# tomguluson92/SCAT

Measured on AMD Instinct MI355X. Metric: images/sec (train step, 256x256 source -> 224x224, reg_transformer), higher is better.
Workload: dtype f32; 1 GPU; ResNet-50 + dim-halving transformer (8 heads) + 3 regressor iterations, pl_reg, mask_rate 0.2, pos_embed, Adam; full train step (BASELINE configs[1]); batch_per_gpu=96, global_batch=96, parallelism=dp1

## Files before the change

### scat_amd/_lib.py

```python
from __future__ import annotations

import ctypes
import os
import re

HERE = os.path.dirname(os.path.abspath(__file__))
HEADER = os.path.join(HERE, "..", "include", "scat_hip.h")
EVAL_HEADER = os.path.join(HERE, "..", "include", "scat_eval.h")
RENDER_HEADER = os.path.join(HERE, "..", "include", "scat_render.h")
MANO_HEADER = os.path.join(HERE, "..", "include", "scat_mano.h")
FIT_HEADER = os.path.join(HERE, "..", "include", "scat_mano_fit.h")
FIT_KP_HEADER = os.path.join(HERE, "..", "include", "scat_mano_fit_kp.h")
HEADERS = (HEADER, EVAL_HEADER, FIT_KP_HEADER, FIT_HEADER, RENDER_HEADER, MANO_HEADER)
LIBPATH = os.path.join(HERE, "libscat_hip.so")
if os.environ.get("SCAT_LIBPATH"):
    import warnings

    LIBPATH = os.path.abspath(os.environ["SCAT_LIBPATH"])
    warnings.warn(f"scat_amd: SCAT_LIBPATH set, loading {LIBPATH} instead of the shipped libscat_hip.so", RuntimeWarning)

_CT = {
    "int": ctypes.c_int,
    "int64_t": ctypes.c_int64,
    "uint64_t": ctypes.c_uint64,
    "float": ctypes.c_float,
}


def parse_header(path: str = HEADER):
    src = open(path).read()
    src = re.sub(r"/\*.*?\*/", "", src, flags=re.S)
    src = re.sub(r"//[^\n]*", "", src)
    protos = {}
    for m in re.finditer(r"(?m)^\s*(const char\*|int64_t|int)\s+(scat_\w+)\s*\(([^;{]*?)\)\s*;", src, flags=re.S):
        ret, name, args = m.group(1), m.group(2), " ".join(m.group(3).split())
        at = []
        if args and args != "void":
            for a in args.split(","):
                a = a.strip()
                if "*" in a:
                    at.append((ctypes.c_void_p, a.split("*")[-1].strip()))
                else:
                    ty, an = a.rsplit(" ", 1)
                    at.append((_CT[ty.replace("const ", "").strip()], an))
        rt = {"int": ctypes.c_int, "int64_t": ctypes.c_int64, "const char*": ctypes.c_char_p}[ret]
        protos[name] = (rt, at)
# ... 53 lines not shown
```

### scat_amd/build.py

```python
from __future__ import annotations

import os
import subprocess
import sys
from concurrent.futures import ThreadPoolExecutor

HERE = os.path.dirname(os.path.abspath(__file__))
CSRC = os.path.join(HERE, "csrc")
OUT = os.path.join(HERE, "libscat_hip.so")
OBJ = os.path.join(HERE, "csrc", "_obj")
HIPCC = os.environ.get("HIPCC", "/opt/rocm/bin/hipcc")
FLAGS = ["-O3", "--offload-arch=gfx950", "-fPIC", "-std=c++17", "-fno-slp-vectorize", "-Wall", "-Wno-unused-function",
         "-Wno-unused-variable"]


def _sources():
    return sorted(f for f in os.listdir(CSRC) if f.endswith(".hip"))


def _public_headers_mtime():
    return max(os.path.getmtime(os.path.join(HERE, "..", "include", h)) for h in ("scat_hip.h", "scat_eval.h", "scat_render.h", "scat_mano.h", "scat_mano_fit.h", "scat_mano_fit_kp.h"))


def _deps_mtime():
    m = 0.0
    for root, _, files in os.walk(CSRC):
        if root.endswith(("_obj", "_obj_diag")):
            continue
        for f in files:
            if f.endswith((".h", ".hip")):
                m = max(m, os.path.getmtime(os.path.join(root, f)))
    return max(m, _public_headers_mtime())


DIAG_OUT = os.path.join(HERE, "..", "tools", "_bin", "libscat_hip_diag.so")


def build(force: bool = False, verbose: bool = True, diag: bool = False) -> str:
    global OUT, OBJ
    if diag:
        out, obj, flags = os.path.abspath(DIAG_OUT), os.path.join(CSRC, "_obj_diag"), FLAGS + ["-DSCAT_DIAG"]
        os.makedirs(os.path.dirname(out), exist_ok=True)
        saved = (OUT, OBJ, list(FLAGS))
        OUT, OBJ = out, obj
        FLAGS[:] = flags
        try:
            return build(force, verbose, False)
        finally:
            OUT, OBJ = saved[0], saved[1]
            FLAGS[:] = saved[2]
    if not force and os.path.exists(OUT) and os.path.getmtime(OUT) >= _deps_mtime():
        return OUT
    os.makedirs(OBJ, exist_ok=True)
    hdr_m = max(os.path.getmtime(os.path.join(CSRC, f)) for f in os.listdir(CSRC) if f.endswith(".h"))
# ... 31 lines not shown
```

### scat_amd/csrc/norm.hip

```cpp
#include <atomic>
#include <chrono>

#include "common.h"

namespace scat {

__device__ __forceinline__ double wave_sum(double v) {
#pragma unroll
    for (int o = 32; o > 0; o >>= 1) v += __shfl_down(v, o, 64);
    return v;
}
__device__ __forceinline__ float wave_sum_f(float v) {
#pragma unroll
    for (int o = 32; o > 0; o >>= 1) v += __shfl_xor(v, o, 64);
    return v;
}

__device__ __forceinline__ void block_sum2(double& a, double& b, double* sh) {
    a = wave_sum(a);
    b = wave_sum(b);
    const int lane = threadIdx.x & 63, w = threadIdx.x >> 6;
    if (lane == 0) { sh[w] = a; sh[4 + w] = b; }
    __syncthreads();
    if (threadIdx.x == 0) {
        a = sh[0] + sh[1] + sh[2] + sh[3];
        b = sh[4] + sh[5] + sh[6] + sh[7];
    }
}

struct BnSlot {
    double s1, s2;
    unsigned long long tag, pad;
};
static std::atomic<unsigned long long> g_bn_tag{1};
static unsigned long long bn_next_tag() {
    static const unsigned long long salt =
// ... 364 lines not shown
    }
}

__global__ __launch_bounds__(256) void bn_bwd_pool_apply_kernel(const float* __restrict__ dyp, const int8_t* __restrict__ idx,
                                                                const float* __restrict__ x, int relu,
                                                                const float* __restrict__ scale,
                                                                const float* __restrict__ shift,
                                                                const float* __restrict__ mean,
                                                                const float* __restrict__ invstd,
                                                                const float* __restrict__ gamma,
                                                                const float* __restrict__ coef, float* __restrict__ dx,
                                                                int64_t total, int C, int W, int OH, int OW) {
    const int QW = OW / 2;
    for (int64_t e = blockIdx.x * 256ll + threadIdx.x; e < total; e += gridDim.x * 256ll) {
        const int b2 = e % QW;
        const int64_t r = e / QW;
        const int a = r % OH;
        const int64_t nc = r / OH;
        const int c = (int)(nc % C);
        const float* g = dyp + nc * OH * OW;
        const int8_t* id = idx + nc * OH * OW;
        const int b = 2 * b2;
        float gv[2][3];
        int iv[2][3];
#pragma unroll
        for (int u = 0; u < 2; ++u)
#pragma unroll
            for (int v = 0; v < 3; ++v) {
                const bool ok = (a + u < OH) && (b + v < OW);
                const int q = ok ? (a + u) * OW + b + v : 0;
                gv[u][v] = ok ? g[q] : 0.f;
                iv[u][v] = ok ? (int)id[q] : -1;
            }
        float top[4], bot[4];
#pragma unroll
        for (int v = 0; v < 2; ++v) {
            top[2 * v] = iv[0][v] == 4 ? gv[0][v] : 0.f;
            top[2 * v + 1] = (iv[0][v] == 5 ? gv[0][v] : 0.f) + (iv[0][v + 1] == 3 ? gv[0][v + 1] : 0.f);
            bot[2 * v] = (iv[0][v] == 7 ? gv[0][v] : 0.f) + (iv[1][v] == 1 ? gv[1][v] : 0.f);
            bot[2 * v + 1] = (iv[0][v] == 8 ? gv[0][v] : 0.f) + (iv[0][v + 1] == 6 ? gv[0][v + 1] : 0.f) +
                             (iv[1][v] == 2 ? gv[1][v] : 0.f) + (iv[1][v + 1] == 0 ? gv[1][v + 1] : 0.f);
        }
        const float sc = scale[c], sh = shift[c], mu = mean[c], is = invstd[c];
        const float k1 = coef[2 * c], k2 = coef[2 * c + 1], gi = gamma[c] * is;
        const int64_t off = (nc * 2 * OH + 2 * a) * W + 2 * b;
        const float4 x0 = *(const float4*)(x + off), x1 = *(const float4*)(x + off + W);
        const float xt[4] = {x0.x, x0.y, x0.z, x0.w}, xb[4] = {x1.x, x1.y, x1.z, x1.w};
        float ot[4], ob[4];
#pragma unroll
        for (int q = 0; q < 4; ++q) {
            const float gt = bn_mask(top[q], xt[q], 0.f, false, relu, sc, sh), gb = bn_mask(bot[q], xb[q], 0.f, false, relu, sc, sh);
            ot[q] = gi * (gt - k1 - (xt[q] - mu) * is * k2);
            ob[q] = gi * (gb - k1 - (xb[q] - mu) * is * k2);
        }
        *(float4*)(dx + off) = make_float4(ot[0], ot[1], ot[2], ot[3]);
        *(float4*)(dx + off + W) = make_float4(ob[0], ob[1], ob[2], ob[3]);
    }
}

template <int V>
__global__ __launch_bounds__(1024) void bn_bwd_reduce_fin_kernel(const float* __restrict__ dy, const float* __restrict__ x,
                                                                 const float* __restrict__ yout,
                                                                 const uint8_t* __restrict__ ymask, int relu,
                                                                 const float* __restrict__ scale,
                                                                 const float* __restrict__ shift,
                                                                 const float* __restrict__ mean,
                                                                 const float* __restrict__ invstd, int B, int C, int HW,
                                                                 FastDiv dHWv, double count, float* __restrict__ dgamma,
                                                                 float* __restrict__ dbeta, float* __restrict__ coef) {
    const int c = blockIdx.x;
    const float sc = scale[c], sh = shift[c], mu = mean[c], is = invstd[c];
    const int hwv = HW / V;
    const bool has_m = V == 4 && ymask != nullptr;
    const bool has_y = yout != nullptr || has_m;
    double s1 = 0, s2 = 0;
    for (int idx = threadIdx.x; idx < B * hwv; idx += 1024) {
        const int n = (int)dHWv.div((uint32_t)idx), i = idx - n * hwv;
        const int64_t off = ((int64_t)n * C + c) * HW + i * V;
        float xv[V], gv[V], yv[V];
        if (V == 4) {
            float4 t = ld4x(x + off); xv[0] = t.x; xv[1] = t.y; xv[2] = t.z; xv[3] = t.w;
            t = *(const float4*)(dy + off); gv[0] = t.x; gv[1] = t.y; gv[2] = t.z; gv[3] = t.w;
            if (has_m) {
                const uint32_t m = ymask[off >> 2];
                yv[0] = (float)(m & 1u); yv[1] = (float)((m >> 1) & 1u); yv[2] = (float)((m >> 2) & 1u); yv[3] = (float)((m >> 3) & 1u);
            } else if (has_y) { t = *(const float4*)(yout + off); yv[0] = t.x; yv[1] = t.y; yv[2] = t.z; yv[3] = t.w; }
// ... 551 lines not shown
                               shift, save_mean, save_invstd, B, C, HW, FastDiv::make(HW / 4), (double)B * HW, dgamma,
                               dbeta, coef);
        else
            hipLaunchKernelGGL(bn_bwd_reduce_fin_kernel<1>, dim3(C), dim3(1024), 0, st, dy, x, y_out, nullptr, relu, scale,
                               shift, save_mean, save_invstd, B, C, HW, FastDiv::make(HW), (double)B * HW, dgamma, dbeta,
                               coef);
    } else {
        BnFin f = bn_fin_base(ws, C, S, (double)B * HW);
        f.dgamma = dgamma; f.dbeta = dbeta; f.coef = coef; f.coef3 = 0;
        if (vec)
            hipLaunchKernelGGL(bn_bwd_reduce_kernel<4>, dim3(C, S), dim3(256), 0, st, dy, x, y_out, y_mask, relu, scale,
                               shift, save_mean, save_invstd, B, C, HW, S, FastDiv::make(HW / 4), part, f);
        else
            hipLaunchKernelGGL(bn_bwd_reduce_kernel<1>, dim3(C, S), dim3(256), 0, st, dy, x, y_out, nullptr, relu, scale,
                               shift, save_mean, save_invstd, B, C, HW, S, FastDiv::make(HW), part, f);
        if (!f.slots)
            hipLaunchKernelGGL(bn_bwd_finalize_kernel, dim3(cdiv(C, 128)), dim3(128), 0, st, (const double*)part, C, S,
                               (double)B * HW, dgamma, dbeta, coef);
    }
    if (vec) {
        const int64_t nv = total / 4;
        hipLaunchKernelGGL(bn_bwd_apply_kernel<4>, dim3(ew_grid(nv)), dim3(256), 0, st, dy, x, y_out, y_mask, relu,
                           scale, shift, save_mean, save_invstd, gamma, (const float*)coef, dx, dres, dres_accumulate, nv,
                           FastDiv::make(HW / 4), FastDiv::make(C), store_policy(total * 4) == 2);
    } else {
        hipLaunchKernelGGL(bn_bwd_apply_kernel<1>, dim3(ew_grid(total)), dim3(256), 0, st, dy, x, y_out, nullptr, relu,
                           scale, shift, save_mean, save_invstd, gamma, (const float*)coef, dx, dres, dres_accumulate, total,
                           FastDiv::make(HW), FastDiv::make(C), 0);
    }
    SCAT_LAUNCH_CHECK("scat_bn_bwd");
    return SCAT_OK;
}

extern "C" int scat_bn_bwd_maxpool(const float* dy_pooled, const int8_t* idx, const float* x, int relu, const float* scale,
                                   const float* shift, const float* save_mean, const float* save_invstd,
                                   const float* gamma, float* dgamma, float* dbeta, float* dx, int B, int C, int H, int W,
                                   void* ws, int64_t ws_bytes, void* stream) {
    SCAT_REQUIRE(dy_pooled && idx && x && scale && shift && save_mean && save_invstd && gamma && dgamma && dbeta && dx,
                 SCAT_E_ARG, "scat_bn_bwd_maxpool: null pointer");
    SCAT_REQUIRE(B > 0 && C > 0 && H > 0 && W > 0 && H % 2 == 0 && W % 4 == 0, SCAT_E_SHAPE,
                 "scat_bn_bwd_maxpool: needs even H and W % 4 == 0");
    SCAT_REQUIRE((((uintptr_t)x | (uintptr_t)dx) & 15) == 0, SCAT_E_SHAPE, "scat_bn_bwd_maxpool: 16-B aligned tensors");
    SCAT_REQUIRE(ws && ws_bytes >= scat_bn_ws(B, C, H * W), SCAT_E_WORKSPACE, "scat_bn_bwd_maxpool: workspace too small");
    SCAT_REQUIRE(((uintptr_t)ws & 7) == 0, SCAT_E_WORKSPACE, "scat_bn_bwd_maxpool: workspace not 8-byte aligned");
    SCAT_REQUIRE(fits_i32((int64_t)B * C * H * W), SCAT_E_SHAPE, "scat_bn_bwd_maxpool: tensor exceeds 2^31 elements");
    const int S = bn_splits(B, C);
    double* part = (double*)ws;
    float* coef = bn_ws_coef(ws, C, S);
    hipStream_t st = (hipStream_t)stream;
    BnFin f = bn_fin_base(ws, C, S, (double)B * H * W);
    f.dgamma = dgamma; f.dbeta = dbeta; f.coef = coef; f.coef3 = 0;
    hipLaunchKernelGGL(bn_bwd_pool_reduce_kernel, dim3(C, S), dim3(256), 0, st, dy_pooled, idx, x, relu, scale, shift, save_mean,
                       save_invstd, B, C, H, W, S, part, f);
    if (!f.slots)
        hipLaunchKernelGGL(bn_bwd_finalize_kernel, dim3(cdiv(C, 128)), dim3(128), 0, st, (const double*)part, C, S,
                           (double)B * H * W, dgamma, dbeta, coef);
    const int OH = H / 2, OW = W / 2;
    const int64_t total = (int64_t)B * C * OH * (OW / 2);
    hipLaunchKernelGGL(bn_bwd_pool_apply_kernel, dim3(ew_grid(total)), dim3(256), 0, st, dy_pooled, idx, x, relu, scale, shift,
                       save_mean, save_invstd, gamma, (const float*)coef, dx, total, C, W, OH, OW);
    SCAT_LAUNCH_CHECK("scat_bn_bwd_maxpool");
    return SCAT_OK;
}

extern "C" int scat_bn_bwd_pre(float* dy_g, const float* dy_add, const float* x, const float* y_out, const uint8_t* y_mask, int relu,
                               const float* scale, const float* shift, const float* save_mean,
                               const float* save_invstd, const float* gamma, float* dgamma, float* dbeta,
                               float* coef3, int B, int C, int HW, void* ws, int64_t ws_bytes, void* stream) {
    SCAT_REQUIRE(dy_g && x && scale && shift && save_mean && save_invstd && gamma && dgamma && dbeta && coef3, SCAT_E_ARG,
                 "scat_bn_bwd_pre: null pointer");
    SCAT_REQUIRE(B > 0 && C > 0 && HW > 0, SCAT_E_SHAPE, "scat_bn_bwd_pre: non-positive dimension");
    SCAT_REQUIRE(ws && ws_bytes >= scat_bn_ws(B, C, HW), SCAT_E_WORKSPACE, "scat_bn_bwd_pre: workspace too small");
    SCAT_REQUIRE(((uintptr_t)ws & 7) == 0, SCAT_E_WORKSPACE, "scat_bn_bwd_pre: workspace not 8-byte aligned");
    SCAT_REQUIRE(!(y_mask && y_out), SCAT_E_ARG, "scat_bn_bwd_pre: pass the output OR its sign mask");
    SCAT_REQUIRE((HW & 3) == 0 && (((uintptr_t)dy_g | (uintptr_t)dy_add | (uintptr_t)x | (uintptr_t)y_out) & 15) == 0, SCAT_E_SHAPE,
                 "scat_bn_bwd_pre: needs HW % 4 == 0 and 16-B aligned tensors");
    SCAT_REQUIRE(fits_i32((int64_t)B * C * HW), SCAT_E_SHAPE, "scat_bn_bwd_pre: tensor exceeds 2^31 elements");
    const int S = bn_splits(B, C);
    double* part = (double*)ws;
    hipStream_t st = (hipStream_t)stream;
    BnFin f = bn_fin_base(ws, C, S, (double)B * HW);
    f.dgamma = dgamma; f.dbeta = dbeta; f.coef = coef3; f.coef3 = 1; f.gamma = gamma; f.mean = save_mean; f.invstd = save_invstd;
    hipLaunchKernelGGL(bn_bwd_reduce_g_kernel, dim3(C, S), dim3(256), 0, st, dy_g, dy_add, x, y_out, y_mask, relu, scale, shift,
                       save_mean, save_invstd, B, C, HW, S, FastDiv::make(HW / 4), part, f);
    if (!f.slots)
        hipLaunchKernelGGL(bn_bwd_finalize3_kernel, dim3(cdiv(C, 128)), dim3(128), 0, st, (const double*)part, C, S,
                           (double)B * HW, gamma, save_mean, save_invstd, dgamma, dbeta, coef3);
    SCAT_LAUNCH_CHECK("scat_bn_bwd_pre");
    return SCAT_OK;
// ... 160 lines not shown
```

### scat_amd/csrc/stem_wgrad.hip

```cpp
#include "conv_common.h"
#include "split.h"

namespace scat {

struct StemWgDesc {
    const float* dy;
    const float* x;
    float* slab;
    int B, H, W, OH, OW;
    int rows;
    int rpw;
    int64_t ndy, nx;
};

constexpr int SW_PW = 232;
constexpr int SW_PATCH = 3 * 7 * SW_PW;

__global__ __launch_bounds__(256) void stem_wgrad_split_kernel(StemWgDesc d) {
    extern __shared__ __align__(16) float lds[];
    const int tid = threadIdx.x, lane = tid & 63, wave = tid >> 6;
    const int l31 = lane & 31, lh = lane >> 5;
    const int rb = wave & 1;
    const int cb0 = (wave >> 1) * 3, ncb = (wave >> 1) ? 2 : 3;
    const int r_beg = blockIdx.x * d.rpw, r_end = min(r_beg + d.rpw, d.rows);

    const __amdgpu_buffer_rsrc_t rsx = make_rsrc(d.x, d.nx), rsy = make_rsrc(d.dy, d.ndy);

    constexpr int NP = (3 * 7 * SW_PW + 255) / 256;
    float pst[NP];
    auto load_patch = [&](int row) {
        const bool live = row < r_end;
        const int n = live ? row / d.OH : 0, oy = live ? row - n * d.OH : 0;
#pragma unroll
        for (int i = 0; i < NP; ++i) {
            const int it = tid + 256 * i;
            const int q = it / SW_PW, v = it - q * SW_PW;
            const int c = q / 7, r = q - 7 * c;
            const int iy = 2 * oy + r - 3, ix = v - 3;
            const bool ok = live && it < SW_PATCH && (unsigned)iy < (unsigned)d.H && (unsigned)ix < (unsigned)d.W;
            pst[i] = __uint_as_float(__builtin_amdgcn_raw_buffer_load_b32(
                rsx, ok ? (((n * 3 + c) * d.H + iy) * d.W + ix) * 4 : OOB, 0, 0));
        }
    };
    auto store_patch = [&](float* dst) {
#pragma unroll
        for (int i = 0; i < NP; ++i) {
            const int it = tid + 256 * i;
            if (it < SW_PATCH) dst[it] = pst[i];
        }
    };

    int boff[3];
    bool bok[3];
#pragma unroll
    for (int t = 0; t < 3; ++t) {
        const int n = (cb0 + t) * 32 + l31;
        bok[t] = t < ncb && n < 147;
        const int nn = bok[t] ? n : 0;
        const int c = nn / 49, kh = (nn - 49 * c) / 7, kw = nn - 49 * c - 7 * kh;
        boff[t] = (c * 7 + kh) * SW_PW + kw + 16 * lh;
    }

    f32x16 acc[3];
#pragma unroll
    for (int t = 0; t < 3; ++t)
#pragma unroll
        for (int r = 0; r < 16; ++r) acc[t][r] = 0.f;

    const int nsteps = d.OW / 16;
    float araw[2][8];
    auto load_a = [&](int row, int step, auto set_tag) {
        constexpr int Q = decltype(set_tag)::value;
        const bool live = row < r_end;
        const int n = live ? row / d.OH : 0, oy = live ? row - n * d.OH : 0;
        const int off = live ? ((((n * 64 + rb * 32 + l31) * d.OH + oy) * d.OW) + 16 * step + 8 * lh) * 4 : OOB;
        const u32x4 t0 = __builtin_amdgcn_raw_buffer_load_b128(rsy, off, 0, 0);
        const u32x4 t1 = __builtin_amdgcn_raw_buffer_load_b128(rsy, off, 16, 0);
#pragma unroll
        for (int e = 0; e < 4; ++e) { araw[Q][e] = __uint_as_float(t0[e]); araw[Q][4 + e] = __uint_as_float(t1[e]); }
    };
    using S0 = std::integral_constant<int, 0>;
    using S1 = std::integral_constant<int, 1>;

    load_patch(r_beg);
    store_patch(lds);
    load_a(r_beg, 0, S0{});
    __syncthreads();
    int pbuf = 0;
    auto row_body = [&](int row, auto p_tag) {
        constexpr int P = decltype(p_tag)::value;
        const float* patch = lds + pbuf * SW_PATCH;
        load_patch(row + 1);
        auto step = [&](int s, auto cur_tag) {
            constexpr int CUR = decltype(cur_tag)::value;
            if (s + 1 < nsteps) load_a(row, s + 1, std::integral_constant<int, CUR ^ 1>{});
            else load_a(row + 1, 0, std::integral_constant<int, CUR ^ 1>{});
            u32x4 a[3];
            split3x8(araw[CUR], a[0], a[1], a[2]);
#pragma unroll
            for (int t = 0; t < 3; ++t) {
                if (t < ncb) {
                    float v[8];
                    const float* p = patch + boff[t] + 32 * s;
#pragma unroll
                    for (int e = 0; e < 8; ++e) v[e] = bok[t] ? p[2 * e] : 0.f;
                    u32x4 b[3];
                    split3x8(v, b[0], b[1], b[2]);
                    acc[t] = mfma_split(a, b, acc[t]);
                }
            }
        };
        for (int s = 0; s < nsteps; s += 2) {
            step(s, std::integral_constant<int, P>{});
            if (s + 1 < nsteps) step(s + 1, std::integral_constant<int, P ^ 1>{});
        }
        store_patch(lds + (pbuf ^ 1) * SW_PATCH);
        pbuf ^= 1;
        __syncthreads();
    };
    int par = 0;
    for (int row = r_beg; row < r_end; ++row) {
        if (par == 0) row_body(row, S0{});
        else row_body(row, S1{});
        par ^= nsteps & 1;
    }

    float* out = d.slab + (int64_t)blockIdx.x * 64 * 147;
#pragma unroll
    for (int t = 0; t < 3; ++t) {
        if (t < ncb) {
            const int n = (cb0 + t) * 32 + l31;
            if (n < 147) {
#pragma unroll
                for (int r = 0; r < 16; ++r) {
                    const int co = rb * 32 + (r & 3) + 8 * (r >> 2) + 4 * lh;
                    out[co * 147 + n] = acc[t][r];
                }
            }
        }
    }
}

}

using namespace scat;

static int stem_wg_rows_per_wg(int rows) {
    int rpw = (rows + 767) / 768;
    if (rpw < 4) rpw = 4;
    return rpw;
}

extern "C" int64_t scat_conv7x7_s2_wgrad_split_ws(int B, int H, int W) {
    const int OH = (H + 6 - 7) / 2 + 1;
    const int rows = B * OH, rpw = stem_wg_rows_per_wg(rows);
    return (int64_t)((rows + rpw - 1) / rpw) * 64 * 147 * 4;
}

extern "C" int scat_conv7x7_s2_wgrad_split(const float* dy, const float* x, float* dw, int B, int H, int W, int Cout,
                                           void* ws, int64_t ws_bytes, void* stream) {
    SCAT_REQUIRE(dy && x && dw, SCAT_E_ARG, "scat_conv7x7_s2_wgrad_split: null pointer");
    SCAT_REQUIRE(math_mode() == 1, SCAT_E_ARG, "scat_conv7x7_s2_wgrad_split: needs the split-operand product mode");
    const int OH = (H + 6 - 7) / 2 + 1, OW = (W + 6 - 7) / 2 + 1;
    SCAT_REQUIRE(B > 0 && Cout == 64 && OW % 16 == 0 && OW <= 112 && 2 * OW + 5 <= SW_PW, SCAT_E_SHAPE,
                 "scat_conv7x7_s2_wgrad_split: Cout = 64, output width a multiple of 16 up to 112 (got Cout %d OW %d)", Cout, OW);
    SCAT_REQUIRE(ws && ws_bytes >= scat_conv7x7_s2_wgrad_split_ws(B, H, W) && ((uintptr_t)ws & 15) == 0 &&
                     ((uintptr_t)dy & 15) == 0,
                 SCAT_E_WORKSPACE, "scat_conv7x7_s2_wgrad_split: workspace too small / unaligned");
    SCAT_REQUIRE(fits_i32((int64_t)B * 64 * OH * OW * 4) && fits_i32((int64_t)B * 3 * H * W * 4), SCAT_E_SHAPE,
                 "scat_conv7x7_s2_wgrad_split: tensor exceeds 32-bit byte offsets");
    hipStream_t st = (hipStream_t)stream;
    StemWgDesc d{};
    d.dy = dy; d.x = x; d.slab = (float*)ws; d.B = B; d.H = H; d.W = W; d.OH = OH; d.OW = OW;
    d.rows = B * OH; d.rpw = stem_wg_rows_per_wg(d.rows);
    d.ndy = (int64_t)B * 64 * OH * OW; d.nx = (int64_t)B * 3 * H * W;
    const int splits = (d.rows + d.rpw - 1) / d.rpw;
    set_kernel_label("wgrad7x7_s2_split_64x160x16_split%d", splits);
    hipLaunchKernelGGL(stem_wgrad_split_kernel, dim3(splits), dim3(256), (size_t)2 * SW_PATCH * 4, st, d);
    SCAT_LAUNCH_CHECK("scat_conv7x7_s2_wgrad_split");
    launch_splitk_reduce((const float*)ws, dw, (int64_t)64 * 147, splits, 0, st);
    SCAT_LAUNCH_CHECK("scat_conv7x7_s2_wgrad_split(reduce)");
    return SCAT_OK;
}
```

### scat_amd/models/resnet.py

```python
from __future__ import annotations

import os

import torch

from .. import _switches as _sw
import torch.nn as nn

from .. import nn as snn
from .. import ops

__all__ = ["ResNet", "Bottleneck", "resnet50", "resnet101", "resnet152"]


class Bottleneck(nn.Module):
    expansion = 4

    def __init__(self, inplanes, planes, stride=1, downsample=None):
        super().__init__()
        self.conv1 = snn.Conv2d(inplanes, planes, kernel_size=1, bias=False)
        self.bn1 = snn.BatchNorm2d(planes)
        self.conv2 = snn.Conv2d(planes, planes, kernel_size=3, stride=stride, padding=1, bias=False)
        self.bn2 = snn.BatchNorm2d(planes)
        self.conv3 = snn.Conv2d(planes, planes * 4, kernel_size=1, bias=False)
# ... 13 lines not shown
_NBT = []
_DEFER = [False]


class _BNState:
    __slots__ = ("mean", "invstd", "scale", "shift", "xs")

    def __init__(self, x, bn, training):
        if training:
            self.mean, self.invstd, self.scale, self.shift = ops.bn_train_stats(
                x, bn.weight, bn.bias, bn.running_mean, bn.running_var, bn.momentum, bn.eps)
            bn._stat_ref = self.mean
            _NBT.append(bn.num_batches_tracked)
            bn._fold_cache = None
        else:
            ver = (bn.weight._version, bn.bias._version, bn.running_mean._version, bn.running_var._version,
                   bn.weight.data_ptr(), bn.running_mean.data_ptr())
            c = getattr(bn, "_fold_cache", None)
            if c is None or c[0] != ver:
                c = (ver, *ops.bn_eval_fold(bn.weight, bn.bias, bn.running_mean, bn.running_var, bn.eps))
                bn._fold_cache = c
            self.scale, self.shift = c[1], c[2]
            self.mean = self.invstd = None


BNB1 = _sw.ab("SCAT_BNB1", False)
BNB1_MIN_H = _sw.ab_int("SCAT_BNB1_MIN_H", 0)
BNB_MIN_H = _sw.ab_int("SCAT_BNB_MIN_H", 28)
BNB = _sw.ab("SCAT_BNB", True)
SUBSAMPLE = _sw.ab("SCAT_SUBSAMPLE", True)
SIDE_SHORTCUT = _sw.ab("SCAT_SIDE_SHORTCUT", True)
SIDE_DS_BN = _sw.ab("SCAT_SIDE_DS_BN", True)
STEM_FUSED_BWD = _sw.ab("SCAT_STEM_FUSED_BWD", True)
SIDE_WGRAD = _sw.ab("SCAT_SIDE_WGRAD", True)
EPI_BNB = _sw.ab("SCAT_EPI_BNB", True)


def _side_stream(device, who="backbone"):
    if not SIDE_WGRAD:
        return None
    from .. import streams
    return streams.get(device, "wgrad" if who == "backbone" else "tokens_wgrad")


STAT_REF = _sw.ab("SCAT_STAT_REF", True)


def _ref(bn):
    return getattr(bn, "_stat_ref", None) if STAT_REF else None


def _block_forward(blk, xin, training, wp=None):
    def shortcut():
        xs = ops.subsample2(xin) if blk.stride == 2 and SUBSAMPLE else None
        if xs is not None:
            cd = ops.conv2d_fwd(xs, blk.downsample[0].weight, 1, 0, wp=wp, stats=training,
                                stats_shift=_ref(blk.downsample[1]))
        else:
            cd = ops.conv2d_fwd(xin, blk.downsample[0].weight, blk.stride, 0, wp=wp, stats=training,
                                stats_shift=_ref(blk.downsample[1]))
        sd = _BNState(cd, blk.downsample[1], training)
        sd.xs = xs if training else None
        return cd, sd

    cd = sd = None
    side = _side_stream(xin.device) if (blk.downsample is not None and SIDE_SHORTCUT and xin.is_cuda) else None
# ... 331 lines not shown
                return dcur if dcur is not None else torch.zeros_like(like)
            if ext is None:
                return dcur if dcur is not None else torch.zeros_like(like)
            ext = ext if ext.is_contiguous() else ext.contiguous()
            if dcur is None:
                return ext.clone()
            return ops.axpy(dcur, ext, 1.0, out=dcur)

        li = lids[-1]
        remaining = len(layers[li])
        dcur = add_ext(dcur, stage_grads[li], x4)
        recs = list(reversed(tape))
        pre3 = None
        for k, rec in enumerate(recs):
            nxt = recs[k + 1] if remaining > 1 and k + 1 < len(recs) else None
            dcur, pre3 = _block_backward(bc, rec, dcur, nxt, pre3)
            remaining -= 1
            if remaining == 0:
                if sink is not None:
                    join()
                    sink.ready(("layer%d" % (li + 1),))
                li -= 1
                if li >= lids[0]:
                    remaining = len(layers[li])
                    dcur = add_ext(dcur, stage_grads[li], dcur)
        if part == 2:
            join()
            ctx.tape = ctx.stem = ctx.tail = None
            net._own_dx2 = dcur.data_ptr()
            if sink is not None:
                return (dcur, None, None, *[None for _ in net._flat_params])
            return (dcur, None, None, *[grads.get(p) for p in net._flat_params])
        x, c0, s0, idx0 = ctx.stem
        if STEM_FUSED_BWD and c0.shape[2] % 2 == 0 and c0.shape[3] % 4 == 0 and dcur.is_contiguous():
            dc0, dg, db = ops.bn_bwd_maxpool(dcur, idx0, c0, True, s0.scale, s0.shift, s0.mean, s0.invstd, net.bn1.weight,
                                             gbuf(net.bn1.weight), gbuf(net.bn1.bias))
        else:
            da0 = ops.maxpool_bwd(dcur, idx0, tuple(c0.shape))
            dc0, dg, db = ops.bn_bwd(da0, c0, None, True, s0.scale, s0.shift, s0.mean, s0.invstd, net.bn1.weight,
                                     gbuf(net.bn1.weight), gbuf(net.bn1.bias), dx=da0)
        put(net.bn1.weight, dg), put(net.bn1.bias, db)
        put(net.conv1.weight, wgrad(dc0, x, net.conv1.weight, 2, 3))
        join()
        ctx.tape = ctx.stem = ctx.tail = None
        if sink is not None:
            sink.ready(("stem",))
            sink.adopt(net._flat_params)
            return (None, None, None, *[None for _ in net._flat_params])
        return (None, None, None, *[grads.get(p) for p in net._flat_params])


class ResNet(nn.Module):
    def __init__(self, block, layers, num_classes=1000):
        self.inplanes = 64
        super().__init__()
        self.conv1 = snn.Conv2d(3, 64, kernel_size=7, stride=2, padding=3, bias=False)
        self.bn1 = snn.BatchNorm2d(64)
        self.relu = snn.ReLU(inplace=True)
        self.maxpool = snn.MaxPool2d(kernel_size=3, stride=2, padding=1)
        self.layer1 = self._make_layer(block, 64, layers[0])
        self.layer2 = self._make_layer(block, 128, layers[1], stride=2)
        self.layer3 = self._make_layer(block, 256, layers[2], stride=2)
        self.layer4 = self._make_layer(block, 512, layers[3], stride=2)
        self.avgpool = snn.AvgPool2d(7)
        self.fc1 = snn.Linear(512 * block.expansion, 1024)
        self._wprep = ops.WeightPrep()
        for m in self.modules():
            if isinstance(m, nn.Conv2d):
                nn.init.kaiming_normal_(m.weight, mode="fan_out", nonlinearity="relu")
            elif isinstance(m, nn.BatchNorm2d):
                nn.init.constant_(m.weight, 1)
                nn.init.constant_(m.bias, 0)
        self._flat_params = None

    def _make_layer(self, block, planes, blocks, stride=1):
# ... 69 lines not shown
```

### scat_amd/ops.py

```python
from __future__ import annotations

import ctypes
import os

import torch

from . import _switches as _sw

from ._lib import ScatError, lib

_ws_cache = {}

PROFILE = None


def _prof(flops, fn, *args):
    if PROFILE is None:
        return fn(*args)
    e0, e1 = torch.cuda.Event(enable_timing=True), torch.cuda.Event(enable_timing=True)
    e0.record()
    r = fn(*args)
    e1.record()
    PROFILE.append((lib().scat_last_kernel().decode(), float(flops), e0, e1))
    return r
# ... 537 lines not shown
def bn_bwd(dy, x, y_out, relu, scale, shift, save_mean, save_invstd, gamma, dgamma=None, dbeta=None, dx=None,
           dres=None, dres_accumulate=False, y_mask=None):
    if y_mask is not None:
        y_out = None
    _chk(dy, x, y_out, scale, shift, save_mean, save_invstd, gamma, dgamma, dbeta, dx, dres)
    B, C, H, W = x.shape
    dx = dx if dx is not None else torch.empty_like(x)
    dgamma = dgamma if dgamma is not None else torch.empty_like(gamma)
    dbeta = dbeta if dbeta is not None else torch.empty_like(gamma)
    ws = workspace(lib().scat_bn_ws(B, C, H * W), x.device)
    sign = 8.0 if y_out is not None else (0.0625 if y_mask is not None else 0.0)
    nb = x.numel() * (8.0 + 12.0 + sign + (4.0 if dres is not None and dres is not dy else 0.0))
    if BN_ONEPASS and C >= 64 and B * H * W // (4 if (H * W) % 4 == 0 else 1) <= 8192:
        nb = x.numel() * (12.0 + sign / 2 + (4.0 if dres is not None and dres is not dy else 0.0))
    _prof_hbm("bn_bwd" + ("_res" if dres is not None else ""), nb, lib().scat_bn_bwd, _p(dy), _p(x), _p(y_out),
              _p(y_mask), int(relu), _p(scale), _p(shift), _p(save_mean), _p(save_invstd), _p(gamma), _p(dgamma),
              _p(dbeta), _p(dx), _p(dres), int(dres_accumulate), B, C, H * W, _p(ws), ws.numel(), _stream())
    return dx, dgamma, dbeta


def bn_bwd_maxpool(dy_pooled, idx, x, relu, scale, shift, save_mean, save_invstd, gamma, dgamma=None, dbeta=None):
    _chk(dy_pooled, x, scale, shift, save_mean, save_invstd, gamma, dgamma, dbeta)
    B, C, H, W = x.shape
    assert tuple(dy_pooled.shape) == (B, C, H // 2, W // 2) and idx.shape == dy_pooled.shape and idx.dtype == torch.int8
    dx = torch.empty_like(x)
    dgamma = dgamma if dgamma is not None else torch.empty_like(gamma)
    dbeta = dbeta if dbeta is not None else torch.empty_like(gamma)
    ws = workspace(lib().scat_bn_ws(B, C, H * W), x.device)
    nb = dy_pooled.numel() * (2 * 5.0 + 4.0) + x.numel() * 8.0
    _prof_hbm("bn_bwd_maxpool", nb, lib().scat_bn_bwd_maxpool, _p(dy_pooled), _p(idx), _p(x), int(relu), _p(scale), _p(shift),
              _p(save_mean), _p(save_invstd), _p(gamma), _p(dgamma), _p(dbeta), _p(dx), B, C, H, W, _p(ws), ws.numel(),
              _stream())
    return dx, dgamma, dbeta


def bn_bwd_pre(dy, x, relu, scale, shift, save_mean, save_invstd, gamma, dgamma=None, dbeta=None, y_out=None,
               y_mask=None, dy_add=None):
    _chk(dy, x, y_out, scale, shift, save_mean, save_invstd, gamma, dgamma, dbeta, dy_add)
    B, C, H, W = x.shape
    dgamma = dgamma if dgamma is not None else torch.empty_like(gamma)
    dbeta = dbeta if dbeta is not None else torch.empty_like(gamma)
    coef3 = torch.empty((3, C), dtype=torch.float32, device=x.device)
    ws = workspace(lib().scat_bn_ws(B, C, H * W), x.device)
    sign = 4.0 if y_out is not None else (0.03125 if y_mask is not None else 0.0)
    nb = x.numel() * (12.0 + sign + (4.0 if dy_add is not None else 0.0))
    _prof_hbm("bn_bwd_pre", nb, lib().scat_bn_bwd_pre, _p(dy), _p(dy_add), _p(x), _p(y_out), _p(y_mask), int(relu),
              _p(scale), _p(shift), _p(save_mean), _p(save_invstd), _p(gamma), _p(dgamma), _p(dbeta), _p(coef3), B, C,
              H * W, _p(ws), ws.numel(), _stream())
    return coef3, dgamma, dbeta


def epilogue_bnb_arm(x, mask, mean):
    _chk(x, mean)
    B, C, H, W = x.shape
    nbytes = C * ((B * H * W + 31) // 32 + 4) * 8
    part = workspace(nbytes, x.device, "bnbpart")
    lib().scat_epilogue_bnb_arm(_p(x), _p(mask), _p(mean), x.numel(), _p(part), nbytes)
    return part


def epilogue_bnb_groups():
    return lib().scat_epilogue_bnb_groups()


def bn_bwd_pre_partials(part, groups, x_shape, save_mean, save_invstd, gamma, dgamma=None, dbeta=None):
    _chk(save_mean, save_invstd, gamma, dgamma, dbeta)
# ... 484 lines not shown
```

Before: 4353 images/s.

## Fuse stem BN+maxpool backward apply into conv1 weight-gradient kernel

```diff
diff --git a/include/scat_stem.h b/include/scat_stem.h
--- /dev/null
+++ b/include/scat_stem.h
@@ -0,0 +1,20 @@
+#ifndef SCAT_STEM_H
+#define SCAT_STEM_H
+#include <stdint.h>
+
+#include "scat_hip.h"
+#ifdef __cplusplus
+extern "C" {
+#endif
+
+int64_t scat_stem_bwd_scratch_bytes(int B, int H, int W);
+
+int scat_stem_bwd(const float* dy_pooled, const int8_t* idx, const float* c0, const float* x,
+                  const float* scale, const float* shift, const float* save_mean, const float* save_invstd,
+                  const float* gamma, float* dgamma, float* dbeta, float* dw,
+                  int B, int H, int W, void* scratch, int64_t scratch_bytes, void* stream);
+
+#ifdef __cplusplus
+}
+#endif
+#endif
diff --git a/scat_amd/_lib.py b/scat_amd/_lib.py
--- a/scat_amd/_lib.py
+++ b/scat_amd/_lib.py
@@ -6,12 +6,13 @@
 
 HERE = os.path.dirname(os.path.abspath(__file__))
 HEADER = os.path.join(HERE, "..", "include", "scat_hip.h")
+STEM_HEADER = os.path.join(HERE, "..", "include", "scat_stem.h")
 EVAL_HEADER = os.path.join(HERE, "..", "include", "scat_eval.h")
 RENDER_HEADER = os.path.join(HERE, "..", "include", "scat_render.h")
 MANO_HEADER = os.path.join(HERE, "..", "include", "scat_mano.h")
 FIT_HEADER = os.path.join(HERE, "..", "include", "scat_mano_fit.h")
 FIT_KP_HEADER = os.path.join(HERE, "..", "include", "scat_mano_fit_kp.h")
-HEADERS = (HEADER, EVAL_HEADER, FIT_KP_HEADER, FIT_HEADER, RENDER_HEADER, MANO_HEADER)
+HEADERS = (HEADER, STEM_HEADER, EVAL_HEADER, FIT_KP_HEADER, FIT_HEADER, RENDER_HEADER, MANO_HEADER)
 LIBPATH = os.path.join(HERE, "libscat_hip.so")
 if os.environ.get("SCAT_LIBPATH"):
     import warnings
diff --git a/scat_amd/build.py b/scat_amd/build.py
--- a/scat_amd/build.py
+++ b/scat_amd/build.py
@@ -19,7 +19,7 @@
 
 
 def _public_headers_mtime():
-    return max(os.path.getmtime(os.path.join(HERE, "..", "include", h)) for h in ("scat_hip.h", "scat_eval.h", "scat_render.h", "scat_mano.h", "scat_mano_fit.h", "scat_mano_fit_kp.h"))
+    return max(os.path.getmtime(os.path.join(HERE, "..", "include", h)) for h in ("scat_hip.h", "scat_stem.h", "scat_eval.h", "scat_render.h", "scat_mano.h", "scat_mano_fit.h", "scat_mano_fit_kp.h"))
 
 
 def _deps_mtime():
diff --git a/scat_amd/csrc/bn_pool_grad.h b/scat_amd/csrc/bn_pool_grad.h
--- /dev/null
+++ b/scat_amd/csrc/bn_pool_grad.h
@@ -0,0 +1,40 @@
+#pragma once
+#include <hip/hip_runtime.h>
+
+namespace scat {
+
+struct BnPoolK {
+    float sc, sh;
+    float mu, is;
+    float gi;
+    float k1, k2;
+};
+
+template <int PX>
+__device__ __forceinline__ float bn_pool_scatter(int py, const float (&g)[2][2], const int (&t)[2][2]) {
+    if (py == 0) {
+        if (PX == 0) return t[0][0] == 4 ? g[0][0] : 0.f;
+        return (t[0][0] == 5 ? g[0][0] : 0.f) + (t[0][1] == 3 ? g[0][1] : 0.f);
+    }
+    if (PX == 0) return (t[0][0] == 7 ? g[0][0] : 0.f) + (t[1][0] == 1 ? g[1][0] : 0.f);
+    return (t[0][0] == 8 ? g[0][0] : 0.f) + (t[0][1] == 6 ? g[0][1] : 0.f) + (t[1][0] == 2 ? g[1][0] : 0.f) +
+           (t[1][1] == 0 ? g[1][1] : 0.f);
+}
+
+template <int PX>
+__device__ __forceinline__ float bn_pool_dx(int py, const float (&g)[2][2], const int (&t)[2][2], float x, int relu,
+                                            const BnPoolK& k) {
+#pragma clang fp contract(off)
+    float gs = bn_pool_scatter<PX>(py, g, t);
+    if (relu) gs = __builtin_fmaf(x, k.sc, k.sh) > 0.f ? gs : 0.f;
+    const float xh = (x - k.mu) * k.is;
+    const float r = __builtin_fmaf(-k.k2, xh, gs - k.k1);
+    return k.gi * r;
+}
+
+const float* launch_bn_bwd_pool_reduce(const float* dy_pooled, const int8_t* idx, const float* x, int relu,
+                                       const float* scale, const float* shift, const float* save_mean,
+                                       const float* save_invstd, float* dgamma, float* dbeta, int B, int C, int H, int W,
+                                       void* ws, hipStream_t st);
+
+}
diff --git a/scat_amd/csrc/norm.hip b/scat_amd/csrc/norm.hip
--- a/scat_amd/csrc/norm.hip
+++ b/scat_amd/csrc/norm.hip
@@ -2,6 +2,7 @@
 #include <chrono>
 
 #include "common.h"
+#include "bn_pool_grad.h"
 
 namespace scat {
 
@@ -432,26 +433,21 @@
                 gv[u][v] = ok ? g[q] : 0.f;
                 iv[u][v] = ok ? (int)id[q] : -1;
             }
-        float top[4], bot[4];
-#pragma unroll
-        for (int v = 0; v < 2; ++v) {
-            top[2 * v] = iv[0][v] == 4 ? gv[0][v] : 0.f;
-            top[2 * v + 1] = (iv[0][v] == 5 ? gv[0][v] : 0.f) + (iv[0][v + 1] == 3 ? gv[0][v + 1] : 0.f);
-            bot[2 * v] = (iv[0][v] == 7 ? gv[0][v] : 0.f) + (iv[1][v] == 1 ? gv[1][v] : 0.f);
-            bot[2 * v + 1] = (iv[0][v] == 8 ? gv[0][v] : 0.f) + (iv[0][v + 1] == 6 ? gv[0][v + 1] : 0.f) +
-                             (iv[1][v] == 2 ? gv[1][v] : 0.f) + (iv[1][v + 1] == 0 ? gv[1][v + 1] : 0.f);
-        }
-        const float sc = scale[c], sh = shift[c], mu = mean[c], is = invstd[c];
-        const float k1 = coef[2 * c], k2 = coef[2 * c + 1], gi = gamma[c] * is;
+        BnPoolK k;
+        k.sc = scale[c]; k.sh = shift[c]; k.mu = mean[c]; k.is = invstd[c];
+        k.k1 = coef[2 * c]; k.k2 = coef[2 * c + 1]; k.gi = gamma[c] * k.is;
         const int64_t off = (nc * 2 * OH + 2 * a) * W + 2 * b;
         const float4 x0 = *(const float4*)(x + off), x1 = *(const float4*)(x + off + W);
         const float xt[4] = {x0.x, x0.y, x0.z, x0.w}, xb[4] = {x1.x, x1.y, x1.z, x1.w};
         float ot[4], ob[4];
 #pragma unroll
-        for (int q = 0; q < 4; ++q) {
-            const float gt = bn_mask(top[q], xt[q], 0.f, false, relu, sc, sh), gb = bn_mask(bot[q], xb[q], 0.f, false, relu, sc, sh);
-            ot[q] = gi * (gt - k1 - (xt[q] - mu) * is * k2);
-            ob[q] = gi * (gb - k1 - (xb[q] - mu) * is * k2);
+        for (int v = 0; v < 2; ++v) {
+            const float g[2][2] = {{gv[0][v], gv[0][v + 1]}, {gv[1][v], gv[1][v + 1]}};
+            const int t[2][2] = {{iv[0][v], iv[0][v + 1]}, {iv[1][v], iv[1][v + 1]}};
+            ot[2 * v] = bn_pool_dx<0>(0, g, t, xt[2 * v], relu, k);
+            ot[2 * v + 1] = bn_pool_dx<1>(0, g, t, xt[2 * v + 1], relu, k);
+            ob[2 * v] = bn_pool_dx<0>(1, g, t, xb[2 * v], relu, k);
+            ob[2 * v + 1] = bn_pool_dx<1>(1, g, t, xb[2 * v + 1], relu, k);
         }
         *(float4*)(dx + off) = make_float4(ot[0], ot[1], ot[2], ot[3]);
         *(float4*)(dx + off + W) = make_float4(ob[0], ob[1], ob[2], ob[3]);
@@ -1069,6 +1065,23 @@
     return SCAT_OK;
 }
 
+const float* scat::launch_bn_bwd_pool_reduce(const float* dy_pooled, const int8_t* idx, const float* x, int relu,
+                                             const float* scale, const float* shift, const float* save_mean,
+                                             const float* save_invstd, float* dgamma, float* dbeta, int B, int C, int H,
+                                             int W, void* ws, hipStream_t st) {
+    const int S = bn_splits(B, C);
+    double* part = (double*)ws;
+    float* coef = bn_ws_coef(ws, C, S);
+    BnFin f = bn_fin_base(ws, C, S, (double)B * H * W);
+    f.dgamma = dgamma; f.dbeta = dbeta; f.coef = coef; f.coef3 = 0;
+    hipLaunchKernelGGL(bn_bwd_pool_reduce_kernel, dim3(C, S), dim3(256), 0, st, dy_pooled, idx, x, relu, scale, shift, save_mean,
+                       save_invstd, B, C, H, W, S, part, f);
+    if (!f.slots)
+        hipLaunchKernelGGL(bn_bwd_finalize_kernel, dim3(cdiv(C, 128)), dim3(128), 0, st, (const double*)part, C, S,
+                           (double)B * H * W, dgamma, dbeta, coef);
+    return coef;
+}
+
 extern "C" int scat_bn_bwd_maxpool(const float* dy_pooled, const int8_t* idx, const float* x, int relu, const float* scale,
                                    const float* shift, const float* save_mean, const float* save_invstd,
                                    const float* gamma, float* dgamma, float* dbeta, float* dx, int B, int C, int H, int W,
@@ -1081,17 +1094,9 @@
     SCAT_REQUIRE(ws && ws_bytes >= scat_bn_ws(B, C, H * W), SCAT_E_WORKSPACE, "scat_bn_bwd_maxpool: workspace too small");
     SCAT_REQUIRE(((uintptr_t)ws & 7) == 0, SCAT_E_WORKSPACE, "scat_bn_bwd_maxpool: workspace not 8-byte aligned");
     SCAT_REQUIRE(fits_i32((int64_t)B * C * H * W), SCAT_E_SHAPE, "scat_bn_bwd_maxpool: tensor exceeds 2^31 elements");
-    const int S = bn_splits(B, C);
-    double* part = (double*)ws;
-    float* coef = bn_ws_coef(ws, C, S);
     hipStream_t st = (hipStream_t)stream;
-    BnFin f = bn_fin_base(ws, C, S, (double)B * H * W);
-    f.dgamma = dgamma; f.dbeta = dbeta; f.coef = coef; f.coef3 = 0;
-    hipLaunchKernelGGL(bn_bwd_pool_reduce_kernel, dim3(C, S), dim3(256), 0, st, dy_pooled, idx, x, relu, scale, shift, save_mean,
-                       save_invstd, B, C, H, W, S, part, f);
-    if (!f.slots)
-        hipLaunchKernelGGL(bn_bwd_finalize_kernel, dim3(cdiv(C, 128)), dim3(128), 0, st, (const double*)part, C, S,
-                           (double)B * H * W, dgamma, dbeta, coef);
+    const float* coef = launch_bn_bwd_pool_reduce(dy_pooled, idx, x, relu, scale, shift, save_mean, save_invstd, dgamma, dbeta,
+                                                  B, C, H, W, ws, st);
     const int OH = H / 2, OW = W / 2;
     const int64_t total = (int64_t)B * C * OH * (OW / 2);
     hipLaunchKernelGGL(bn_bwd_pool_apply_kernel, dim3(ew_grid(total)), dim3(256), 0, st, dy_pooled, idx, x, relu, scale, shift,
diff --git a/scat_amd/csrc/stem_wgrad.hip b/scat_amd/csrc/stem_wgrad.hip
--- a/scat_amd/csrc/stem_wgrad.hip
+++ b/scat_amd/csrc/stem_wgrad.hip
@@ -1,5 +1,6 @@
 #include "conv_common.h"
 #include "split.h"
+#include "bn_pool_grad.h"
 
 namespace scat {
 
@@ -11,12 +12,20 @@
     int rows;
     int rpw;
     int64_t ndy, nx;
+    const float* dyp;
+    const int8_t* idx;
+    const float *scale, *shift, *mean, *invstd, *gamma;
+    const float* coef;
 };
 
 constexpr int SW_PW = 232;
 constexpr int SW_PATCH = 3 * 7 * SW_PW;
-
-__global__ __launch_bounds__(256) void stem_wgrad_split_kernel(StemWgDesc d) {
+constexpr int SW_DYP = 116;
+constexpr int SW_ITEMS = (64 * 14 + 255) / 256;
+constexpr int SW_LDS_BNPOOL = (2 * SW_PATCH + 64 * SW_DYP + 7 * 64) * 4;
+
+template <bool BNPOOL>
+__device__ __forceinline__ void stem_wgrad_body(const StemWgDesc& d) {
     extern __shared__ __align__(16) float lds[];
     const int tid = threadIdx.x, lane = tid & 63, wave = tid >> 6;
     const int l31 = lane & 31, lh = lane >> 5;
@@ -82,21 +91,118 @@
     using S0 = std::integral_constant<int, 0>;
     using S1 = std::integral_constant<int, 1>;
 
+    float* dyrow = lds + 2 * SW_PATCH;
+    float* kst = dyrow + 64 * SW_DYP;
+    const int PH = d.OH / 2, PW = d.OW / 2, nk = d.OW / 8;
+    __amdgpu_buffer_rsrc_t rsg = rsy, rsi = rsy;
+    if (BNPOOL) {
+        const int64_t np = (int64_t)d.B * 64 * PH * PW;
+        rsg = make_rsrc(d.dyp, np);
+        rsi = __builtin_amdgcn_make_buffer_rsrc((void*)d.idx, 0, (int)np, 0x00020000);
+        if (tid < 64) {
+            const float is = d.invstd[tid];
+            kst[tid] = d.scale[tid]; kst[64 + tid] = d.shift[tid]; kst[128 + tid] = d.mean[tid]; kst[192 + tid] = is;
+            kst[256 + tid] = d.gamma[tid] * is; kst[320 + tid] = d.coef[2 * tid]; kst[384 + tid] = d.coef[2 * tid + 1];
+        }
+        __syncthreads();
+    }
+    u32x4 xraw[SW_ITEMS][2];
+    auto load_c0 = [&](int row) {
+        const bool live = row < r_end;
+        const int n = live ? row / d.OH : 0, oy = live ? row - n * d.OH : 0;
+#pragma unroll
+        for (int j = 0; j < SW_ITEMS; ++j) {
+            const int i = tid + 256 * j;
+            const bool ok = live && i < 64 * nk;
+            const int ch = ok ? i / nk : 0, k = ok ? i - ch * nk : 0;
+            const int off = ok ? (((n * 64 + ch) * d.OH + oy) * d.OW + 8 * k) * 4 : OOB;
+            xraw[j][0] = __builtin_amdgcn_raw_buffer_load_b128(rsy, off, 0, 0);
+            xraw[j][1] = __builtin_amdgcn_raw_buffer_load_b128(rsy, off, 16, 0);
+        }
+    };
+    auto form_item = [&](int n, int oy, int i, const u32x4& x0, const u32x4& x1, auto py_tag) {
+        constexpr int py = decltype(py_tag)::value;
+        const bool ok = i < 64 * nk;
+        const int ch = ok ? i / nk : 0, k = ok ? i - ch * nk : 0;
+        const int p0 = ((n * 64 + ch) * PH + (oy >> 1)) * PW + 4 * k;
+        const bool cok = ok && 4 * k + 4 < PW;
+        float gr[2][5];
+        uint32_t tr[2][2];
+#pragma unroll
+        for (int u = 0; u <= py; ++u) {
+            const bool rok = ok && (u == 0 || (oy >> 1) + 1 < PH);
+            const int p = p0 + u * PW;
+            const u32x4 g4 = __builtin_amdgcn_raw_buffer_load_b128(rsg, rok ? p * 4 : OOB, 0, 0);
+#pragma unroll
+            for (int e = 0; e < 4; ++e) gr[u][e] = __uint_as_float(g4[e]);
+            gr[u][4] = __uint_as_float(__builtin_amdgcn_raw_buffer_load_b32(rsg, rok && cok ? (p + 4) * 4 : OOB, 0, 0));
+            tr[u][0] = __builtin_amdgcn_raw_buffer_load_b32(rsi, rok ? p : OOB, 0, 0);
+            tr[u][1] = __builtin_amdgcn_raw_buffer_load_b8(rsi, rok && cok ? p + 4 : OOB, 0, 0);
+        }
+        if (py == 0) {
+#pragma unroll
+            for (int e = 0; e < 5; ++e) gr[1][e] = 0.f;
+            tr[1][0] = tr[1][1] = 0u;
+        }
+        BnPoolK bk;
+        bk.sc = kst[ch]; bk.sh = kst[64 + ch]; bk.mu = kst[128 + ch]; bk.is = kst[192 + ch];
+        bk.gi = kst[256 + ch]; bk.k1 = kst[320 + ch]; bk.k2 = kst[384 + ch];
+        float av[8];
+#pragma unroll
+        for (int q = 0; q < 4; ++q) {
+            float g[2][2];
+            int t[2][2];
+#pragma unroll
+            for (int u = 0; u < 2; ++u)
+#pragma unroll
+                for (int v = 0; v < 2; ++v) {
+                    g[u][v] = gr[u][q + v];
+                    t[u][v] = q + v < 4 ? (int)((tr[u][0] >> (8 * (q + v))) & 0xffu) : (int)(tr[u][1] & 0xffu);
+                }
+            const float xe = __uint_as_float(q < 2 ? x0[2 * q] : x1[2 * q - 4]);
+            const float xo = __uint_as_float(q < 2 ? x0[2 * q + 1] : x1[2 * q - 3]);
+            av[2 * q] = bn_pool_dx<0>(py, g, t, xe, 1, bk);
+            av[2 * q + 1] = bn_pool_dx<1>(py, g, t, xo, 1, bk);
+        }
+        if (ok) {
+            float4* dst = (float4*)(dyrow + ch * SW_DYP + 8 * k);
+            dst[0] = make_float4(av[0], av[1], av[2], av[3]);
+            dst[1] = make_float4(av[4], av[5], av[6], av[7]);
+        }
+    };
+    auto form_row = [&](int row) {
+        const int n = row / d.OH, oy = row - n * d.OH;
+#pragma unroll
+        for (int j = 0; j < SW_ITEMS; ++j) {
+            if (oy & 1) form_item(n, oy, tid + 256 * j, xraw[j][0], xraw[j][1], S1{});
+            else form_item(n, oy, tid + 256 * j, xraw[j][0], xraw[j][1], S0{});
+        }
+    };
+
     load_patch(r_beg);
     store_patch(lds);
-    load_a(r_beg, 0, S0{});
+    if (BNPOOL) { load_c0(r_beg); form_row(r_beg); }
+    else load_a(r_beg, 0, S0{});
     __syncthreads();
     int pbuf = 0;
     auto row_body = [&](int row, auto p_tag) {
         constexpr int P = decltype(p_tag)::value;
         const float* patch = lds + pbuf * SW_PATCH;
         load_patch(row + 1);
+        if (BNPOOL) load_c0(row + 1);
         auto step = [&](int s, auto cur_tag) {
             constexpr int CUR = decltype(cur_tag)::value;
-            if (s + 1 < nsteps) load_a(row, s + 1, std::integral_constant<int, CUR ^ 1>{});
-            else load_a(row + 1, 0, std::integral_constant<int, CUR ^ 1>{});
             u32x4 a[3];
-            split3x8(araw[CUR], a[0], a[1], a[2]);
+            if (BNPOOL) {
+                const float4* ap = (const float4*)(dyrow + (rb * 32 + l31) * SW_DYP + 16 * s + 8 * lh);
+                const float4 a0 = ap[0], a1 = ap[1];
+                const float av[8] = {a0.x, a0.y, a0.z, a0.w, a1.x, a1.y, a1.z, a1.w};
+                split3x8(av, a[0], a[1], a[2]);
+            } else {
+                if (s + 1 < nsteps) load_a(row, s + 1, std::integral_constant<int, CUR ^ 1>{});
+                else load_a(row + 1, 0, std::integral_constant<int, CUR ^ 1>{});
+                split3x8(araw[CUR], a[0], a[1], a[2]);
+            }
 #pragma unroll
             for (int t = 0; t < 3; ++t) {
                 if (t < ncb) {
@@ -116,11 +222,15 @@
         }
         store_patch(lds + (pbuf ^ 1) * SW_PATCH);
         pbuf ^= 1;
+        if (BNPOOL) {
+            __syncthreads();
+            if (row + 1 < r_end) form_row(row + 1);
+        }
         __syncthreads();
     };
     int par = 0;
     for (int row = r_beg; row < r_end; ++row) {
-        if (par == 0) row_body(row, S0{});
+        if (par == 0 || BNPOOL) row_body(row, S0{});
         else row_body(row, S1{});
         par ^= nsteps & 1;
     }
@@ -140,6 +250,9 @@
         }
     }
 }
+
+__global__ __launch_bounds__(256) void stem_wgrad_split_kernel(StemWgDesc d) { stem_wgrad_body<false>(d); }
+__global__ __launch_bounds__(256, 2) void stem_wgrad_bnpool_kernel(StemWgDesc d) { stem_wgrad_body<true>(d); }
 
 }
 
@@ -182,3 +295,53 @@
     SCAT_LAUNCH_CHECK("scat_conv7x7_s2_wgrad_split(reduce)");
     return SCAT_OK;
 }
+
+#include "../../include/scat_stem.h"
+
+static int64_t stem_bn_bytes(int B, int OH, int OW) { return (scat_bn_ws(B, 64, OH * OW) + 15) & ~(int64_t)15; }
+
+extern "C" int64_t scat_stem_bwd_scratch_bytes(int B, int H, int W) {
+    if (B <= 0 || H <= 0 || W <= 0) return 0;
+    const int OH = (H + 6 - 7) / 2 + 1, OW = (W + 6 - 7) / 2 + 1;
+    return stem_bn_bytes(B, OH, OW) + scat_conv7x7_s2_wgrad_split_ws(B, H, W);
+}
+
+extern "C" int scat_stem_bwd(const float* dy_pooled, const int8_t* idx, const float* c0, const float* x,
+                             const float* scale, const float* shift, const float* save_mean, const float* save_invstd,
+                             const float* gamma, float* dgamma, float* dbeta, float* dw, int B, int H, int W,
+                             void* scratch, int64_t scratch_bytes, void* stream) {
+    SCAT_REQUIRE(dy_pooled && idx && c0 && x && scale && shift && save_mean && save_invstd && gamma && dgamma && dbeta && dw,
+                 SCAT_E_ARG, "scat_stem_bwd: null pointer");
+    SCAT_REQUIRE(math_mode() == 1, SCAT_E_ARG, "scat_stem_bwd: needs the split-operand product mode");
+    SCAT_REQUIRE(B > 0 && H > 0 && W > 0, SCAT_E_SHAPE, "scat_stem_bwd: non-positive dimension");
+    const int OH = (H + 6 - 7) / 2 + 1, OW = (W + 6 - 7) / 2 + 1;
+    SCAT_REQUIRE(OW % 16 == 0 && OW <= 112 && 2 * OW + 5 <= SW_PW && OH % 2 == 0, SCAT_E_SHAPE,
+                 "scat_stem_bwd: output width a multiple of 16 up to 112, even output height (got OH %d OW %d)", OH, OW);
+    SCAT_REQUIRE((((uintptr_t)c0 | (uintptr_t)dy_pooled) & 15) == 0 && ((uintptr_t)idx & 3) == 0, SCAT_E_SHAPE,
+                 "scat_stem_bwd: c0 and dy_pooled 16-byte aligned, idx 4-byte aligned");
+    SCAT_REQUIRE(fits_i32((int64_t)B * 64 * OH * OW * 4) && fits_i32((int64_t)B * 3 * H * W * 4), SCAT_E_SHAPE,
+                 "scat_stem_bwd: tensor exceeds 32-bit byte offsets");
+    SCAT_REQUIRE(scratch && scratch_bytes >= scat_stem_bwd_scratch_bytes(B, H, W) && ((uintptr_t)scratch & 15) == 0,
+                 SCAT_E_WORKSPACE, "scat_stem_bwd: scratch too small / unaligned");
+    hipStream_t st = (hipStream_t)stream;
+    StemWgDesc d{};
+    d.dy = c0; d.x = x; d.slab = (float*)((char*)scratch + stem_bn_bytes(B, OH, OW));
+    d.B = B; d.H = H; d.W = W; d.OH = OH; d.OW = OW;
+    d.rows = B * OH; d.rpw = stem_wg_rows_per_wg(d.rows);
+    d.ndy = (int64_t)B * 64 * OH * OW; d.nx = (int64_t)B * 3 * H * W;
+    d.dyp = dy_pooled; d.idx = idx; d.scale = scale; d.shift = shift; d.mean = save_mean; d.invstd = save_invstd;
+    d.gamma = gamma;
+    d.coef = launch_bn_bwd_pool_reduce(dy_pooled, idx, c0, 1, scale, shift, save_mean, save_invstd, dgamma, dbeta, B, 64,
+                                       OH, OW, scratch, st);
+    SCAT_LAUNCH_CHECK("scat_stem_bwd(reduce)");
+    const int splits = (d.rows + d.rpw - 1) / d.rpw;
+    set_kernel_label("wgrad7x7_s2_split_64x160x16_bnpool_split%d", splits);
+    static bool once = (hipFuncSetAttribute((const void*)stem_wgrad_bnpool_kernel, hipFuncAttributeMaxDynamicSharedMemorySize,
+                                            SW_LDS_BNPOOL) == hipSuccess);
+    (void)once;
+    hipLaunchKernelGGL(stem_wgrad_bnpool_kernel, dim3(splits), dim3(256), (size_t)SW_LDS_BNPOOL, st, d);
+    SCAT_LAUNCH_CHECK("scat_stem_bwd");
+    launch_splitk_reduce(d.slab, dw, (int64_t)64 * 147, splits, 0, st);
+    SCAT_LAUNCH_CHECK("scat_stem_bwd(slab reduce)");
+    return SCAT_OK;
+}
diff --git a/scat_amd/models/resnet.py b/scat_amd/models/resnet.py
--- a/scat_amd/models/resnet.py
+++ b/scat_amd/models/resnet.py
@@ -69,6 +69,7 @@
 SIDE_SHORTCUT = _sw.ab("SCAT_SIDE_SHORTCUT", True)
 SIDE_DS_BN = _sw.ab("SCAT_SIDE_DS_BN", True)
 STEM_FUSED_BWD = _sw.ab("SCAT_STEM_FUSED_BWD", True)
+STEM_FUSED_WGRAD = _sw.ab("SCAT_STEM_FUSED_WGRAD", True)
 SIDE_WGRAD = _sw.ab("SCAT_SIDE_WGRAD", True)
 EPI_BNB = _sw.ab("SCAT_EPI_BNB", True)
 
@@ -466,7 +467,12 @@
                 return (dcur, None, None, *[None for _ in net._flat_params])
             return (dcur, None, None, *[grads.get(p) for p in net._flat_params])
         x, c0, s0, idx0 = ctx.stem
-        if STEM_FUSED_BWD and c0.shape[2] % 2 == 0 and c0.shape[3] % 4 == 0 and dcur.is_contiguous():
+        dc0 = None
+        if (STEM_FUSED_WGRAD and STEM_FUSED_BWD and ops.STEM_SPLIT and dcur.is_contiguous()
+                and ops.stem_bwd_ok(dcur, idx0, c0, x)):
+            dw0, dg, db = ops.stem_bwd(dcur, idx0, c0, x, s0.scale, s0.shift, s0.mean, s0.invstd, net.bn1.weight,
+                                       gbuf(net.bn1.weight), gbuf(net.bn1.bias), gbuf(net.conv1.weight))
+        elif STEM_FUSED_BWD and c0.shape[2] % 2 == 0 and c0.shape[3] % 4 == 0 and dcur.is_contiguous():
             dc0, dg, db = ops.bn_bwd_maxpool(dcur, idx0, c0, True, s0.scale, s0.shift, s0.mean, s0.invstd, net.bn1.weight,
                                              gbuf(net.bn1.weight), gbuf(net.bn1.bias))
         else:
@@ -474,7 +480,7 @@
             dc0, dg, db = ops.bn_bwd(da0, c0, None, True, s0.scale, s0.shift, s0.mean, s0.invstd, net.bn1.weight,
                                      gbuf(net.bn1.weight), gbuf(net.bn1.bias), dx=da0)
         put(net.bn1.weight, dg), put(net.bn1.bias, db)
-        put(net.conv1.weight, wgrad(dc0, x, net.conv1.weight, 2, 3))
+        put(net.conv1.weight, dw0 if dc0 is None else wgrad(dc0, x, net.conv1.weight, 2, 3))
         join()
         ctx.tape = ctx.stem = ctx.tail = None
         if sink is not None:
diff --git a/scat_amd/ops.py b/scat_amd/ops.py
--- a/scat_amd/ops.py
+++ b/scat_amd/ops.py
@@ -593,6 +593,30 @@
               _p(save_mean), _p(save_invstd), _p(gamma), _p(dgamma), _p(dbeta), _p(dx), B, C, H, W, _p(ws), ws.numel(),
               _stream())
     return dx, dgamma, dbeta
+
+
+def stem_bwd(dy_pooled, idx, c0, x, scale, shift, save_mean, save_invstd, gamma, dgamma=None, dbeta=None, dw=None):
+    _chk(dy_pooled, c0, x, scale, shift, save_mean, save_invstd, gamma, dgamma, dbeta, dw)
+    B, _, H, W = x.shape
+    _, C, OH, OW = c0.shape
+    assert tuple(dy_pooled.shape) == (B, C, OH // 2, OW // 2) and idx.shape == dy_pooled.shape and idx.dtype == torch.int8
+    assert idx.is_contiguous()
+    dgamma = dgamma if dgamma is not None else torch.empty_like(gamma)
+    dbeta = dbeta if dbeta is not None else torch.empty_like(gamma)
+    dw = dw if dw is not None else torch.empty((C, 3, 7, 7), dtype=torch.float32, device=x.device)
+    ws = workspace(lib().scat_stem_bwd_scratch_bytes(B, H, W), x.device)
+    _prof(2.0 * B * OH * OW * C * 3 * 7 * 7, lib().scat_stem_bwd, _p(dy_pooled), _p(idx), _p(c0), _p(x), _p(scale), _p(shift),
+          _p(save_mean), _p(save_invstd), _p(gamma), _p(dgamma), _p(dbeta), _p(dw), B, H, W, _p(ws), ws.numel(), _stream())
+    return dw, dgamma, dbeta
+
+
+def stem_bwd_ok(dy_pooled, idx, c0, x):
+    B, C, OH, OW = c0.shape
+    return (C == 64 and x.shape[1] == 3 and (OH, OW) == conv_out_hw(x.shape[2], x.shape[3], 7, 2, 3)
+            and OW % 16 == 0 and OW <= 112 and OH % 2 == 0 and dy_pooled.is_contiguous() and idx.is_contiguous()
+            and c0.data_ptr() % 16 == 0 and dy_pooled.data_ptr() % 16 == 0 and idx.data_ptr() % 4 == 0
+            and B * 64 * OH * OW * 4 < 2 ** 31 and x.numel() * 4 < 2 ** 31
+            and lib().scat_get_math_mode() == 1)
 
 
 def bn_bwd_pre(dy, x, relu, scale, shift, save_mean, save_invstd, gamma, dgamma=None, dbeta=None, y_out=None,
```

New measurement: 4366 images/s, median of 6. Within noise of the previous version (+0.3%).
